# Princic-1837592/julia-raytracer

Measured on AMD Instinct MI355X. Metric: Mrays/s + wall-clock render time, cornellbox 1280×720×256spp, higher is better.
Workload: dtype f32; 1 GPU; cornellbox path 1280x720x256spp; scene=cornellbox, sampler=path, width=1280, height=720, spp=256, bounces=8, batch=256, traversal=near, traversal_requested=auto, bvh=middle, parallelism=1 tile groups x 1 sample ranges + RCCL reduce

## Files before the change

julia-raytracer_amd/csrc/jt_kernels.h:

```cpp
#pragma once

#include <hip/hip_runtime.h>

#include <algorithm>

#include "jt_bsdf.h"
#include "jt_device.h"
#include "jt_push.h"

#ifndef JT_STAMPS
#define JT_STAMPS 0
#endif
#ifndef JT_NODE_REPEAT_NONE
#define JT_NODE_REPEAT_NONE 4
#endif
#ifndef JT_NODE_REPEAT
#define JT_NODE_REPEAT 3
#endif
#ifndef JT_FIRST_POP_NONE
#define JT_FIRST_POP_NONE 1
#endif
#ifndef JT_FIRST_POP
#define JT_FIRST_POP 2
#endif
// ... 1026 lines not shown
    p[9 * BLOCK] = p[9 * BLOCK] * omw + tn.z * aw;
}

template <int F, class AovT>
__device__ __forceinline__ bool path_hit(const DScene& S, const DParams& P, Path& st, Hit isec, const AovT& aov,
                                         unsigned& shades) {
    if (!isec.hit) {
        if (st.bounce() > 0 || !P.envhidden)
            st.set_radiance<F>(st.radiance<F>() + st.weight<F>() * eval_environment<F>(S, st.d));
        return true;
    }
    bool in_volume = false;
    if ((F & FT_VOL) && st.flag(F_VOLUME)) {
        float rl = rand1f(st.rng), rd = rand1f(st.rng);
        float distance = sample_transmittance(st.vol.density, isec.t, rl, rd);
        v3 tr = eval_transmittance(st.vol.density, distance);
        float tp = sample_transmittance_pdf(st.vol.density, distance, isec.t);
        st.set_weight<F>((st.weight<F>() * tr) / tp);
        in_volume = distance < isec.t;
        isec.t = distance;
    }
    if (!in_volume) {
        v3 outgoing = -st.d;
        Shading sh;
        eval_shading<F>(S, isec.inst, isec.elem, V2(isec.u, isec.v), outgoing, sh);
        shades++;
        if (P.nocaustics) {
            st.set_max_roughness<F>(jl_max(sh.mat.roughness, st.max_roughness<F>()));
            sh.mat.roughness = st.max_roughness<F>();
        }
        if ((F & FT_OPAC) && sh.mat.opacity < 1 && rand1f(st.rng) >= sh.mat.opacity) {
            if (st.opbounce() > 128) return true;
            st.ctl += 1u << CTL_OPB;
            st.o = sh.position + st.d * 0.01f;
            return next_bounce_retry(P, st);
        }
        if (st.bounce() == 0) {
            st.set_flag(F_HIT);
            aov_update<F>(aov, sh.mat.color, sh.normal);
        }
        st.set_radiance<F>(st.radiance<F>() + st.weight<F>() * (dot(sh.normal, outgoing) >= 0 ? sh.mat.emission : V3(0, 0, 0)));
        v3 incoming;
        const bool delta = is_delta(sh.mat);
        if (!delta) {
            if (rand1f(st.rng) < 0.5f) {
                float rnl = rand1f(st.rng);
                v2 rn = rand2f(st.rng);
                incoming = sample_bsdfcos<F>(sh.mat, sh.normal, outgoing, rnl, rn);
            } else {
                float rl = rand1f(st.rng), rel = rand1f(st.rng);
                v2 ruv = rand2f(st.rng);
                incoming = sample_lights<F>(S, sh.position, rl, rel, ruv);
            }
            if (is_zero(incoming)) return true;
#if JT_FUSED_BSDF
            v3 fb;
            float pbv;
            eval_bsdfcos_pdf<F>(sh.mat, sh.normal, outgoing, incoming, fb, pbv);
            st.set_weight<F>(st.weight<F>() * fb);
            st.set_pb<F>(pbv);
#else
            st.set_weight<F>(st.weight<F>() * eval_bsdfcos<F>(sh.mat, sh.normal, outgoing, incoming));
            st.set_pb<F>(sample_bsdfcos_pdf<F>(sh.mat, sh.normal, outgoing, incoming));
#endif
        } else {
            float rnl = rand1f(st.rng);
            incoming = sample_delta<F>(sh.mat, sh.normal, outgoing, rnl);
            v3 f = eval_delta<F>(sh.mat, sh.normal, outgoing, incoming);
            float pd = sample_delta_pdf<F>(sh.mat, sh.normal, outgoing, incoming);
            st.set_weight<F>((st.weight<F>() * f) / pd);
        }
        const int mtype = sh.mat.type;
        if ((F & FT_VOL) && (mtype == M_REFRACTIVE || mtype == M_VOLUMETRIC || mtype == M_SUBSURFACE) &&
            dot(sh.normal, outgoing) * dot(sh.normal, incoming) < 0) {
            if (!st.flag(F_VOLUME)) {
                st.set_flag(F_VOLUME);
                st.vol.density = sh.mat.density;
                st.vol.scattering = sh.mat.scattering;
                st.vol.scanisotropy = sh.mat.scanisotropy;
            } else {
                st.clear_flag(F_VOLUME);
            }
        }
        st.o = sh.position;
        st.d = incoming;
        return delta ? after_weight<F>(P, st) : begin_light_pdf<F>(S, P, st);
    }
    v3 outgoing = -st.d;
    v3 position = st.o + st.d * isec.t;
    v3 incoming;
    if (rand1f(st.rng) < 0.5f) {
        (void)rand1f(st.rng);
        v2 rn = rand2f(st.rng);
        incoming = sample_scattering(st.vol, outgoing, rn);
    } else {
        float rl = rand1f(st.rng), rel = rand1f(st.rng);
        v2 ruv = rand2f(st.rng);
        incoming = sample_lights<F>(S, position, rl, rel, ruv);
    }
    if (is_zero(incoming)) return true;
    st.set_weight<F>(st.weight<F>() * eval_scattering(st.vol, outgoing, incoming));
    st.set_pb<F>(sample_scattering_pdf(st.vol, outgoing, incoming));
    st.o = position;
    st.d = incoming;
    return begin_light_pdf<F>(S, P, st);
}

template <int F, class AovT>
__device__ __forceinline__ bool naive_hit(const DScene& S, const DParams& P, Path& st, Hit isec, const AovT& aov,
                                          unsigned& shades) {
    if (!isec.hit) {
        if (st.bounce() > 0 || !P.envhidden)
            st.set_radiance<F>(st.radiance<F>() + st.weight<F>() * eval_environment<F>(S, st.d));
        return true;
    }
    v3 outgoing = -st.d;
    Shading sh;
    eval_shading<F>(S, isec.inst, isec.elem, V2(isec.u, isec.v), outgoing, sh);
    shades++;
    if ((F & FT_OPAC) && sh.mat.opacity < 1 && rand1f(st.rng) >= sh.mat.opacity) {
        if (st.opbounce() > 128) return true;
        st.ctl += 1u << CTL_OPB;
        st.o = sh.position + st.d * 0.01f;
        return next_bounce_retry(P, st);
    }
    if (st.bounce() == 0) {
        st.set_flag(F_HIT);
        aov_update<F>(aov, sh.mat.color, sh.normal);
    }
    st.set_radiance<F>(st.radiance<F>() + st.weight<F>() * (dot(sh.normal, outgoing) >= 0 ? sh.mat.emission : V3(0, 0, 0)));
    v3 incoming, f;
    float p;
    if (sh.mat.roughness != 0) {
        float rnl = rand1f(st.rng);
        v2 rn = rand2f(st.rng);
        incoming = sample_bsdfcos<F>(sh.mat, sh.normal, outgoing, rnl, rn);
        if (is_zero(incoming)) return true;
#if JT_FUSED_BSDF
        eval_bsdfcos_pdf<F>(sh.mat, sh.normal, outgoing, incoming, f, p);
#else
        f = eval_bsdfcos<F>(sh.mat, sh.normal, outgoing, incoming);
        p = sample_bsdfcos_pdf<F>(sh.mat, sh.normal, outgoing, incoming);
#endif
    } else {
        float rnl = rand1f(st.rng);
        incoming = sample_delta<F>(sh.mat, sh.normal, outgoing, rnl);
        if (is_zero(incoming)) return true;
        f = eval_delta<F>(sh.mat, sh.normal, outgoing, incoming);
        p = sample_delta_pdf<F>(sh.mat, sh.normal, outgoing, incoming);
    }
    st.set_weight<F>((st.weight<F>() * f) / p);
    st.o = sh.position;
    st.d = incoming;
    return after_weight<F>(P, st);
}

__device__ __forceinline__ void eval_camera(const DCamera& cam, v2 image_uv, v2 lens_uv, v3& ro, v3& rd) {
    const fr3 frame = frame_from(cam.frame);
    const v2 film = V2(cam.film_x, cam.film_y);
    if (!cam.orthographic) {
        v3 q = V3(film.x * (0.5f - image_uv.x), film.y * (image_uv.y - 0.5f), cam.lens);
        v3 dc = -normalize(q);
        v3 e = V3(lens_uv.x * cam.aperture / 2, lens_uv.y * cam.aperture / 2, 0);
        v3 p = (dc * cam.focus) / __builtin_fabsf(dc.z);
        v3 d = normalize(p - e);
        ro = transform_point(frame, e);
        rd = transform_direction(frame, d);
    } else {
        float scale = 1 / cam.lens;
        v3 q = V3(film.x * (0.5f - image_uv.x) * scale, film.y * (image_uv.y - 0.5f) * scale, cam.lens);
        v3 e = V3(-q.x, -q.y, 0) + V3(lens_uv.x * cam.aperture / 2, lens_uv.y * cam.aperture / 2, 0);
        v3 p = V3(-q.x, -q.y, -cam.focus);
        v3 d = normalize(p - e);
        ro = transform_point(frame, e);
        rd = transform_direction(frame, d);
    }
}

template <int F>
__device__ __forceinline__ void start_path(const DParams& P, int i, int j, int pixel, int sample, Path& st) {
    st.rng = rng_init(P.seed, pixel, sample);
    v2 puv = rand2f(st.rng);
    v2 luv = rand2f(st.rng);
    v2 uv;
    if (!P.tentfilter) {
        uv = V2(((float)i + puv.x) / (float)P.width, ((float)j + puv.y) / (float)P.height);
    } else {
        const float width = 2.0f, offset = 0.5f;
        v2 fuv = V2(width * (puv.x < 0.5f ? __builtin_sqrtf(2 * puv.x) - 1 : 1 - __builtin_sqrtf(2 - 2 * puv.x)) + offset,
                    width * (puv.y < 0.5f ? __builtin_sqrtf(2 * puv.y) - 1 : 1 - __builtin_sqrtf(2 - 2 * puv.y)) + offset);
        uv = V2(((float)i + fuv.x) / (float)P.width, ((float)j + fuv.y) / (float)P.height);
    }
    eval_camera(P.cam, uv, P.cam.pinhole ? sample_disk_signs(luv) : sample_disk(luv), st.o, st.d);
    st.set_radiance<F>(V3(0, 0, 0));
    st.set_weight<F>(V3(1, 1, 1));
    st.set_max_roughness<F>(0.0f);
    st.ctl = 0u;
    st.phase = PH_SCENE;
}

__device__ __forceinline__ int lane_count(unsigned long long m) {
    return __builtin_popcount((unsigned)m) + __builtin_popcount((unsigned)(m >> 32));
}

__device__ __forceinline__ unsigned wave_sum(unsigned v) {
    for (int off = 32; off > 0; off >>= 1) v += __shfl_xor(v, off, 64);
    return v;
}

struct DAccum {
    float4* image;
    float4* albedo;
    float4* normal;
    long long* hits;
    unsigned long long* counters;
    unsigned* work;
    float4* part_img;
    float4* part_alb;
    float4* part_nrm;
    int nslot;
};

struct KArgs {
    DScene S;
    DParams P;
    int s_begin, s_end;
    DAccum A;
};
#ifndef JT_KARG_RELOAD
#define JT_KARG_RELOAD 1
#endif
template <int F>
__host__ __device__ constexpr bool karg_reload() {
    return JT_KARG_RELOAD && (F & ~(FT_LINL | FT_NOIL)) != (FT_TEX | FT_ATTR | FT_MAT | FT_OPAC | FT_XFORM | FT_ENV | FT_QUAD);
}
template <class T>
__device__ __forceinline__ T karg(size_t off) {
    typedef __attribute__((address_space(4))) const char* kptr;
    kptr p = (kptr)__builtin_amdgcn_kernarg_segment_ptr();
    asm volatile("" : "+s"(p));
    return *(const __attribute__((address_space(4))) T*)(p + off);
}
#ifndef JT_KARG_SCENE
#define JT_KARG_SCENE 1
#endif
template <bool NCACHE, int F>
__host__ __device__ constexpr bool karg_scene() {
    return NCACHE && JT_KARG_SCENE && (F & ~(FT_LINL | FT_NOIL)) != (FT_TEX | FT_ATTR | FT_MAT | FT_OPAC | FT_XFORM);
}
template <bool FROM_KARG>
__device__ __forceinline__ const DScene& shade_scene(const DScene& S) {
    if constexpr (FROM_KARG) {
        typedef __attribute__((address_space(4))) const char* kptr;
        kptr p = (kptr)__builtin_amdgcn_kernarg_segment_ptr();
        asm volatile("" : "+s"(p));
        return *(const DScene*)(const __attribute__((address_space(4))) DScene*)(p + offsetof(KArgs, S));
    } else {
        return S;
    }
}
#ifndef JT_KARG_PARAMS
#define JT_KARG_PARAMS 1
#endif
template <int SAMPLER, int F>
__host__ __device__ constexpr bool karg_params_on() {
    return JT_KARG_PARAMS && SAMPLER == 1 && (F & ~(FT_LINL | FT_NOIL)) != (FT_TEX | FT_ATTR | FT_MAT | FT_OPAC | FT_XFORM);
}
template <bool FROM_KARG>
__device__ __forceinline__ const DParams& karg_params(const DParams& P) {
    if constexpr (FROM_KARG) {
        typedef __attribute__((address_space(4))) const char* kptr;
        kptr p = (kptr)__builtin_amdgcn_kernarg_segment_ptr();
        asm volatile("" : "+s"(p));
        return *(const DParams*)(const __attribute__((address_space(4))) DParams*)(p + offsetof(KArgs, P));
    } else {
        return P;
    }
}
#ifndef JT_KARG_SCENE_LDS
#define JT_KARG_SCENE_LDS 1
#endif
__device__ __forceinline__ DScene blob_scene(const DScene& S, const uint4* blob);
__host__ __device__ constexpr size_t lds_stack_bytes(bool ovf, int ring, int need);
template <bool NCACHE, int RING, bool OVF, int F>
__device__ __forceinline__ DScene shade_scene_lds(const DScene& S0) {
    if constexpr (!NCACHE && JT_KARG_SCENE_LDS) {
        extern __shared__ uint4 dyn_lds[];
        const DScene& K = shade_scene<true>(S0);
        return blob_scene(K, dyn_lds + lds_stack_bytes(OVF, RING, K.stack_need) / 16);
    } else {
        return S0;
    }
}
#define JT_A(f) (karg_reload<F>() ? karg<decltype(DAccum::f)>(offsetof(KArgs, A) + offsetof(DAccum, f)) : A.f)
#define JT_SB (karg_reload<F>() ? karg<int>(offsetof(KArgs, s_begin)) : s_begin)
#define JT_SE (karg_reload<F>() ? karg<int>(offsetof(KArgs, s_end)) : s_end)

constexpr int NBANDS = 8, BAND_STRIDE = 16;

__host__ __device__ __forceinline__ int launch_tiles(const DParams& P) {
    return plan_tiles(P.width, P.height, P.tile_stride, P.tile_offset);
}

#ifndef JT_ITEM_FIRST_POP
#define JT_ITEM_FIRST_POP 2
#endif
template <bool WIDE, int F>
__host__ __device__ constexpr bool item_first_pop() {
    return JT_ITEM_FIRST_POP == 1 || (JT_ITEM_FIRST_POP == 2 && !WIDE && !ft_none(F));
}
constexpr unsigned ITEM_NONE = 0xffffffffu;

__device__ __forceinline__ int item_pixel(unsigned item, const DParams& P, int tiles_x) {
    const int t = (int)(item >> 6), l = (int)(item & 63u);
    return ((t / tiles_x) * 8 + (l >> 3)) * P.width + (t % tiles_x) * 8 + (l & 7);
}
__host__ __device__ __forceinline__ int item_slot(unsigned item, const DParams& P) {
    const int t = (int)(item >> 6);
    float inv = 1.0f / (float)P.tile_stride;
#if defined(__HIP_DEVICE_COMPILE__)
    inv = __uint_as_float(__builtin_amdgcn_readfirstlane(__float_as_uint(inv)));
#endif
    const int u = (int)((float)(t - P.tile_offset) * inv + 0.5f);
    return u * 64 + (int)(item & 63u);
}
__device__ __forceinline__ float stream_weight(const DParams& P, int s) {
    return 1.0f / (float)(((s - P.first) >> P.lk) + 1);
}

#if JT_STAMPS
#define JT_STAMP(x) x
#else
#define JT_STAMP(x)
#endif

template <int SAMPLER, int RING, bool OVF, int COUNT, int F, bool NCACHE, bool WIDE>
__device__ __forceinline__ void trace_body_items(const DScene& S0, const DParams& P0, int s_begin, int s_end,
                                                 const DAccum& A, int* stack) {
    const DScene& S = S0;
    const DParams& P = P0;
    static_assert(lane_lds(F), "the per-lane item body keeps the lane's sample index in LDS");
    const int lane = threadIdx.x & 63;
    const int oslot = (int)blockIdx.x * BLOCK + (int)threadIdx.x;
    if constexpr ((F & (FT_TEX | FT_ENV)) != 0) {
        for (int k = threadIdx.x; k < 512; k += BLOCK) tex_lut[k] = k < 256 ? S.srgb_lut[k] : S.byte_lut[k - 256];
        __syncthreads();
    }
    Counters cnt{0, 0, 0, 0};
    constexpr bool WC = !ft_none(F);
    unsigned w_paths = 0, w_rays = 0, w_lq = 0;
    __shared__ unsigned wave_cnt[WC ? 1 : (BLOCK / 64) * 4];
    unsigned* const wcnt = wave_cnt + (WC ? 0 : (threadIdx.x >> 6) * 4);
    if (!WC && lane < 3) wcnt[lane] = 0u;
    auto lds_count = [&](int k, bool c) {
        if (c) __hip_atomic_fetch_add(wcnt + k, 1u, __ATOMIC_RELAXED, __HIP_MEMORY_SCOPE_WORKGROUP);
    };
    __shared__ float acc_lds[acc_slots(F) * BLOCK];
    float* acc = acc_lds + threadIdx.x;
    int* const acc_i = reinterpret_cast<int*>(acc);
#if JT_STAMPS
    unsigned long long t_trav = 0, t_shade = 0, n_trav = 0, n_shade = 0, lanes_p = 0, lanes_n = 0, steps_p = 0, steps_n = 0;
    unsigned long long t_hit = 0, t_fin = 0, t_qb = 0, n_phit = 0, n_fin = 0, idle = 0, n_mph = 0, n_mty = 0, n_mid = 0;
    unsigned long long lanes_sh = 0, lanes_hit = 0, t_start = 0, n_start = 0, lanes_start = 0;
#endif
    const int tiles_x = (P.width + 7) / 8, tiles = launch_tiles(P);
    const int kstr = 1 << P.lk;
    const int nq = s_end - s_begin < kstr ? s_end - s_begin : kstr;
    unsigned xcc;
    asm volatile("s_getreg_b32 %0, hwreg(HW_REG_XCC_ID)" : "=s"(xcc));
    int band_k = 0;
    int ut = 0, uq = 0, bnext = 64;
    bool drained = false;
    unsigned item = ITEM_NONE;
    bool next_sample = false;
    Aov aov{acc, 0.0f, P.first, P.lk};
    Path st;
    st.pk = acc + acc_base_slots(F) * BLOCK;
    Trav T;
    T.sp = -1;
    T.nprim = 0;
    T.nxt = W_EMPTY;
    for (;;) {
        JT_STAMP(const unsigned long long ts0 = __builtin_amdgcn_s_memtime());
        bool start = next_sample;
        for (;;) {
            const unsigned long long needm = __builtin_amdgcn_ballot_w64(item == ITEM_NONE);
            if (!needm || drained) break;
            if (bnext >= 64) {
                const int band = (int)((xcc + (unsigned)band_k) & (NBANDS - 1));
                constexpr int STRIP = JT_BAND_STRIP;
                const int gx = tiles_x % P.tile_stride == 0 ? tiles_x / P.tile_stride : 0;
                const bool strips = STRIP > 1 && gx > 0;
                const int tiles_y = (P.height + 7) / 8;
                const int bt0 = strips ? band * tiles_y / NBANDS * gx : band * tiles / NBANDS;
                const int bn = strips ? (band + 1) * tiles_y / NBANDS * gx - bt0 : (band + 1) * tiles / NBANDS - bt0;
                unsigned unit = 0;
                if (lane == 0) unit = atomicAdd(JT_A(work) + band * BAND_STRIDE, 1u);
                unit = __builtin_amdgcn_readfirstlane(unit);
                if (unit >= (unsigned)bn * (unsigned)nq) {
                    if (++band_k >= NBANDS) drained = true;
                    continue;
                }
                uq = (int)(unit % (unsigned)nq);
                const int tu = (int)(unit / (unsigned)nq);
                int tile = bt0 + tu;
                if (strips) {
                    const int rows = bn / gx, sidx = tu / (STRIP * gx);
                    const int v = tu - sidx * STRIP * gx, h = rows - sidx * STRIP < STRIP ? rows - sidx * STRIP : STRIP;
                    tile = bt0 + (sidx * STRIP + v % h) * gx + v / h;
                }
                ut = tile * P.tile_stride + P.tile_offset;
                bnext = 0;
            }
            const int nneed = lane_count(needm), take = nneed < 64 - bnext ? nneed : 64 - bnext;
            const int rank = (int)__builtin_amdgcn_mbcnt_hi((unsigned)(needm >> 32), __builtin_amdgcn_mbcnt_lo((unsigned)needm, 0u));
            if (item == ITEM_NONE && rank < take) {
                const int l = bnext + rank;
                const int i = (ut % tiles_x) * 8 + (l & 7), j = (ut / tiles_x) * 8 + (l >> 3);
                if (i < P.width && j < P.height) {
                    item = (unsigned)(ut * 64 + l);
                    start = true;
                    const int s = JT_SB + uq;
                    acc_i[11 * BLOCK] = s;
                    const int pixel = j * P.width + i;
                    float4 im = make_float4(0, 0, 0, 0), al = im, nr = im;
                    int h = 0;
                    if (s - P.first >= kstr) {
                        if (P.lk == 0) {
                            im = JT_A(image)[pixel];
                            al = JT_A(albedo)[pixel];
                            nr = JT_A(normal)[pixel];
                            h = (int)JT_A(hits)[pixel];
                        } else {
                            const size_t o = (size_t)((s - P.first) & (kstr - 1)) * (size_t)JT_A(nslot) +
                                             (size_t)item_slot(item, P);
                            im = JT_A(part_img)[o];
                            al = JT_A(part_alb)[o];
                            nr = JT_A(part_nrm)[o];
                            h = __float_as_int(al.w);
                        }
                    }
                    acc[0] = im.x;
                    acc[BLOCK] = im.y;
                    acc[2 * BLOCK] = im.z;
                    acc[3 * BLOCK] = im.w;
                    acc[4 * BLOCK] = al.x;
                    acc[5 * BLOCK] = al.y;
                    acc[6 * BLOCK] = al.z;
                    acc[7 * BLOCK] = nr.x;
                    acc[8 * BLOCK] = nr.y;
                    acc[9 * BLOCK] = nr.z;
                    acc_i[10 * BLOCK] = h;
                }
            }
            bnext += take;
        }
        next_sample = false;
        if (start) {
            const int sample = acc_i[11 * BLOCK];
            const int pixel = item_pixel(item, P, tiles_x);
            if (!ft_none(F)) acc[12 * BLOCK] = stream_weight(P, sample);
            const DParams& P = karg_params<karg_params_on<SAMPLER, F>()>(P0);
            start_path<F>(P, pixel % P.width, pixel / P.width, pixel, sample, st);
            query_start<WIDE>(S, T, st.o, st.d, -1, stack);
            if (!WC) lds_count(1, true);
            if constexpr (item_first_pop<WIDE, F>()) {
#pragma unroll
                for (int k = 0; k < (!ft_none(F) && (F & FT_LINL) ? JT_FIRST_POP : JT_FIRST_POP_NONE); k++)
                    if (wants_node<WIDE>(T)) node_step_any<WIDE, RING, OVF, COUNT, NCACHE, F>(S, T, stack, oslot, cnt);
            }
        }
        if (WC) w_rays += lane_count(__builtin_amdgcn_ballot_w64(start));
#if JT_STAMPS
        const unsigned long long ts1 = __builtin_amdgcn_s_memtime();
        t_start += ts1 - ts0;
        n_start++;
        lanes_start += lane_count(__builtin_amdgcn_ballot_w64(start));
#endif
        if (__builtin_amdgcn_ballot_w64(item != ITEM_NONE) == 0) break;
        constexpr bool LSTEP = light_steps(SAMPLER, F);
        for (;;) {
            const bool wantp = T.nprim > 0;
            const bool wantn = wants_node<WIDE>(T);
            const bool waiting = query_done<WIDE>(T);
            const int np = lane_count(__builtin_amdgcn_ballot_w64(wantp));
            const int nn = lane_count(__builtin_amdgcn_ballot_w64(wantn));
            int nw = lane_count(__builtin_amdgcn_ballot_w64(waiting));
            const int nb = np + nn;
            if (LSTEP && !S.light_inline) {
                const bool wantl = waiting && st.phase == PH_LIGHT;
                const int nl = lane_count(__builtin_amdgcn_ballot_w64(wantl));
                if (nl > 0 && (nl >= P.light_lanes || nb == 0)) {
                    bool c_lq = false, c_ray = false;
                    if (wantl && rerun_tie<WIDE>(S, T, st.o, st.d, S.lights[st.li].instance, stack)) {
                    } else if (wantl) {
                        if (light_hit<F>(S, P, st, query_hit(T))) {
                            st.phase = PH_FINISH;
                        } else if (st.phase == PH_LIGHT) {
                            if (WC) c_lq = true;
                            else lds_count(2, true);
                            query_start<WIDE>(S, T, st.o, st.d, S.lights[st.li].instance, stack);
                        } else {
                            if (WC) c_ray = true;
                            else lds_count(1, true);
                            query_start<WIDE>(S, T, st.o, st.d, -1, stack);
                        }
                    }
                    if (WC) {
                        w_lq += lane_count(__builtin_amdgcn_ballot_w64(c_lq));
                        w_rays += lane_count(__builtin_amdgcn_ballot_w64(c_ray));
                    }
                    continue;
                }
                nw -= nl;
            }
            if (nb == 0 || nw >= (nb + nw < P.wait_lanes ? nb + nw : P.wait_lanes)) break;
#if JT_STAMPS
            n_trav++;
            idle += 64 - lane_count(__builtin_amdgcn_ballot_w64(item != ITEM_NONE));
            if (np * JT_VOTE_P >= nn * JT_VOTE_N) { steps_p++; lanes_p += np; } else { steps_n++; lanes_n += nn; }
#endif
            if (JT_RAY_FROM_PATH && !(F & FT_XFORM)) {
                T.lo = st.o;
                T.ld = st.d;
            }
            if (np * JT_VOTE_P >= nn * JT_VOTE_N) {
                if (T.nprim > 0) prim_step<COUNT, F>(S, T, cnt);
            } else {
                constexpr int NREP = ft_none(F) ? JT_NODE_REPEAT_NONE : JT_NODE_REPEAT;
#pragma unroll
                for (int k = 0; k < NREP; k++)
                    if (wants_node<WIDE>(T)) node_step_any<WIDE, RING, OVF, COUNT, NCACHE, F>(S, T, stack, oslot, cnt);
            }
        }
#if JT_STAMPS
        const unsigned long long ts2 = __builtin_amdgcn_s_memtime();
        t_trav += ts2 - ts1;
        n_shade++;
        lanes_sh += lane_count(__builtin_amdgcn_ballot_w64(query_done<WIDE>(T)));
        {
            int mid = -1, mt = -1;
            if (query_done<WIDE>(T) && st.phase == PH_SCENE && T.h_inst >= 0) {
                mid = S.inst_shade[T.h_inst].material;
                mt = (F & FT_MAT) ? S.materials[mid].type : (int)M_MATTE;
            }
            if (__builtin_amdgcn_ballot_w64(mt >= 0)) {
                n_mph++;
                lanes_hit += lane_count(__builtin_amdgcn_ballot_w64(mt >= 0));
                for (int ty = 0; ty <= (int)M_GLTFPBR; ty++) n_mty += __builtin_amdgcn_ballot_w64(mt == ty) ? 1u : 0u;
                bool counted = mt < 0;
                for (;;) {
                    const unsigned long long m = __builtin_amdgcn_ballot_w64(!counted);
                    if (!m) break;
                    const int v = __shfl(mid, __ffsll((long long)m) - 1);
                    counted = counted || mid == v;
                    n_mid++;
                }
            }
        }
        unsigned long long ts3 = ts2, ts4 = ts2;
#endif
        constexpr bool LINL = (F & (FT_LINL | FT_NOIL)) != 0;
        {
            const bool tie = query_done<WIDE>(T) && (T.nh & (TIE_SEEN | REF_RERUN)) == TIE_SEEN &&
                             !(LSTEP && st.phase == PH_FINISH);
            if (S.order_flip && __builtin_amdgcn_ballot_w64(tie))
                if (tie) rerun_tie<WIDE>(S, T, st.o, st.d, SAMPLER == 1 && !LINL && st.phase == PH_LIGHT ? S.lights[st.li].instance : -1, stack);
        }
        bool c_path = false, c_lq = false, c_ray = false;
        unsigned n_inl = 0;
        if (query_done<WIDE>(T)) {
            const DParams& P = karg_params<karg_params_on<SAMPLER, F>()>(P0);
            const DScene SL = shade_scene_lds<NCACHE, RING, OVF, F>(S0);
            const DScene& S = NCACHE ? shade_scene<karg_scene<NCACHE, F>()>(S0) : SL;
            bool alive = true;
            const bool light = SAMPLER == 1 && !LINL && st.phase == PH_LIGHT;
            bool done;
            if (LSTEP && st.phase == PH_FINISH) done = true;
            else if (light) done = light_hit<F>(S, P, st, query_hit(T));
            else if (SAMPLER == 2) done = naive_hit<F>(S, P, st, query_hit(T), aov, cnt.shades);
            else done = path_hit<F>(S, P, st, query_hit(T), aov, cnt.shades);
            bool chained = false;
            if (SAMPLER == 1 && !done && st.phase == PH_LIGHT && chains_inline(F, S)) {
                unsigned nlq = 0;
                chained = true;
                done = light_chain<WIDE, RING, OVF, COUNT, NCACHE, F>(S, P, st, T, stack, oslot, cnt, [&] {
                    if (WC) nlq++;
                    else lds_count(2, true);
                });
                if (WC) n_inl += nlq;
            }
#if JT_STAMPS
            ts3 = __builtin_amdgcn_s_memtime();
            n_phit++;
#endif
            if (done) {
                if (WC) c_path = true;
                else lds_count(0, true);
                v3 radiance = st.radiance<F>();
                if (!all_finite(radiance)) radiance = V3(0, 0, 0);
                const float mr = max3(radiance);
                if (mr > P.clamp) radiance = radiance * (P.clamp / mr);
                const float w = aov.w<F>();
                const float omw = 1 - w;
                const bool hit = st.flag(F_HIT);
                const bool env = !hit && !P.envhidden && S.nenvs != 0;
                const v4 target = (hit || env) ? V4(radiance.x, radiance.y, radiance.z, 1) : V4(0, 0, 0, 0);
                if (!hit) aov_update<F>(aov, env ? V3(1, 1, 1) : V3(0, 0, 0), -st.d);
                acc[0] = acc[0] * omw + target.x * w;
                acc[BLOCK] = acc[BLOCK] * omw + target.y * w;
                acc[2 * BLOCK] = acc[2 * BLOCK] * omw + target.z * w;
                acc[3 * BLOCK] = acc[3 * BLOCK] * omw + target.w * w;
                if (hit || env) acc_i[10 * BLOCK] += 1;
                alive = false;
                T.sp = -1;
                const int sample = acc_i[11 * BLOCK];
                if (sample + kstr >= JT_SE) {
                    const int pixel = item_pixel(item, P, tiles_x);
                    const float4 im = make_float4(acc[0], acc[BLOCK], acc[2 * BLOCK], acc[3 * BLOCK]);
                    if (P.lk == 0) {
                        JT_A(image)[pixel] = im;
                        JT_A(albedo)[pixel] = make_float4(acc[4 * BLOCK], acc[5 * BLOCK], acc[6 * BLOCK], 0.0f);
                        JT_A(normal)[pixel] = make_float4(acc[7 * BLOCK], acc[8 * BLOCK], acc[9 * BLOCK], 0.0f);
                        JT_A(hits)[pixel] = (long long)acc_i[10 * BLOCK];
                    } else {
                        const size_t o = (size_t)((sample - P.first) & (kstr - 1)) * (size_t)JT_A(nslot) +
                                         (size_t)item_slot(item, P);
                        JT_A(part_img)[o] = im;
                        JT_A(part_alb)[o] = make_float4(acc[4 * BLOCK], acc[5 * BLOCK], acc[6 * BLOCK], __int_as_float(acc_i[10 * BLOCK]));
                        JT_A(part_nrm)[o] = make_float4(acc[7 * BLOCK], acc[8 * BLOCK], acc[9 * BLOCK], 0.0f);
                    }
                    item = ITEM_NONE;
                } else {
                    acc_i[11 * BLOCK] = sample + kstr;
                    next_sample = true;
                }
            }
#if JT_STAMPS
            ts4 = __builtin_amdgcn_s_memtime();
            if (__builtin_amdgcn_ballot_w64(done)) n_fin++;
#endif
            if (alive) {
                if (SAMPLER == 1 && !LINL && st.phase == PH_LIGHT) {
                    if (WC) c_lq = true;
                    else lds_count(2, true);
                    query_start<WIDE>(S, T, st.o, st.d, S.lights[st.li].instance, stack);
                } else {
                    if (WC) c_ray = true;
                    else lds_count(1, true);
                    if (SAMPLER == 1 && chain_dinv_once<WIDE, OVF, NCACHE, F>() && __builtin_amdgcn_ballot_w64(!chained) == 0)
                        query_restart<F>(S, T, st.o, st.d, stack);
                    else query_start<WIDE>(S, T, st.o, st.d, -1, stack);
                }
#pragma unroll
                for (int k = 0; k < (!ft_none(F) && (F & FT_LINL) ? JT_FIRST_POP : JT_FIRST_POP_NONE); k++)
                    if (wants_node<WIDE>(T)) node_step_any<WIDE, RING, OVF, COUNT, NCACHE, F>(S, T, stack, oslot, cnt);
            }
        }
#if JT_STAMPS
        const unsigned long long ts5 = __builtin_amdgcn_s_memtime();
        t_shade += ts5 - ts2;
        t_hit += ts3 - ts2;
        t_fin += ts4 - ts3;
        t_qb += ts5 - ts4;
#endif
        if (WC) {
            w_paths += lane_count(__builtin_amdgcn_ballot_w64(c_path));
            w_lq += lane_count(__builtin_amdgcn_ballot_w64(c_lq));
            w_rays += lane_count(__builtin_amdgcn_ballot_w64(c_ray));
            if (SAMPLER == 1 && chains_inline(F, S)) w_lq += __builtin_amdgcn_readfirstlane(wave_sum(n_inl));
        }
    }
#if JT_STAMPS
    if (lane == 0) {
        unsigned long long* dbg = A.counters + 8;
        const unsigned long long v[24] = {t_trav, t_shade, n_trav,  n_shade, lanes_p, lanes_n,  steps_p, steps_n,
                                          0,      t_hit,   t_fin,   t_qb,    0,       n_phit,   n_fin,   idle,
                                          n_mph,  n_mty,   n_mid,   lanes_sh, lanes_hit, t_start, n_start, lanes_start};
        for (int k = 0; k < 24; k++) atomicAdd(dbg + k, v[k]);
    }
#endif
    const unsigned wv[3] = {w_paths, w_rays, w_lq};
    unsigned v[7] = {0u, 0u, 0u, cnt.nodes, cnt.instances, cnt.prims, COUNT ? cnt.shades : 0u};
#pragma unroll
    for (int k = 0; k < 7; k++) {
        unsigned sum = k < 3 ? (WC ? wv[k] : wcnt[k]) : wave_sum(v[k]);
        if (lane == 0 && sum) atomicAdd(&A.counters[k], (unsigned long long)sum);
    }
}

struct DCombine {
    float w[JT_MAX_STREAMS];
    int ns;
};
inline void combine_weights(long long n, int lk, DCombine& cw) {
    cw = DCombine{};
    cw.ns = combine_weights(n, lk, cw.w);
}
#ifndef JT_WAVES
#define JT_WAVES 0
#endif
#ifndef JT_WAVES_NONE
#define JT_WAVES_NONE 5
#endif
#if JT_WAVES > 0
#define JT_WAVES_PER_EU __attribute__((amdgpu_waves_per_eu(JT_WAVES, JT_WAVES)))
#define JT_WAVES_PER_EU_F(F) \
    __attribute__((amdgpu_waves_per_eu(ft_none(F) ? JT_WAVES_NONE : JT_WAVES, ft_none(F) ? JT_WAVES_NONE : JT_WAVES)))
#else
#define JT_WAVES_PER_EU
#define JT_WAVES_PER_EU_F(F)
#endif
__host__ __device__ constexpr size_t lds_stack_bytes(bool ovf, int ring, int need) {
    return (size_t)(ovf ? ring : need) * BLOCK * 4;
}

__device__ __forceinline__ DScene blob_scene(const DScene& S, const uint4* blob) {
    DScene L = S;
    L.nodes = reinterpret_cast<const DNode*>(blob + S.o_nodes);
    L.wnodes = reinterpret_cast<const DWide*>(blob + S.o_wnodes);
    L.prims = reinterpret_cast<const float4*>(blob + S.o_prims);
    L.inst_trav = reinterpret_cast<const DInstTrav*>(blob + S.o_inst_trav);
    L.inst_blas = reinterpret_cast<const int4*>(blob + S.o_inst_blas);
    L.inst_shade = reinterpret_cast<const DInstShade*>(blob + S.o_inst_shade);
    L.shapes = reinterpret_cast<const DShape*>(blob + S.o_shapes);
    L.pos = reinterpret_cast<const float4*>(blob + S.o_pos);
    L.nrm = reinterpret_cast<const float4*>(blob + S.o_nrm);
    L.tc = reinterpret_cast<const float2*>(blob + S.o_tc);
    L.col = reinterpret_cast<const float4*>(blob + S.o_col);
    L.elems = reinterpret_cast<const int4*>(blob + S.o_elems);
    L.enrm = reinterpret_cast<const float4*>(blob + S.o_enrm);
    L.enrm_id = reinterpret_cast<const float4*>(blob + S.o_enrm_id);
    L.materials = reinterpret_cast<const DMaterial*>(blob + S.o_materials);
    L.lights = reinterpret_cast<const DLight*>(blob + S.o_lights);
    L.light_hit = reinterpret_cast<const int4*>(blob + S.o_light_hit);
    L.light_elems = reinterpret_cast<const float4*>(blob + S.o_light_elems);
    L.cdf = reinterpret_cast<const float*>(blob + S.o_cdf);
    return L;
}

template <int SAMPLER, int RING, bool OVF, int COUNT, int F, bool WIDE>
__global__ __launch_bounds__(BLOCK) JT_WAVES_PER_EU void trace_kernel(DScene S, DParams P, int s_begin, int s_end, DAccum A) {
    __shared__ int lds_stack[RING * BLOCK];
    trace_body_items<SAMPLER, RING, OVF, COUNT, F, true, WIDE>(S, P, s_begin, s_end, A, lds_stack + threadIdx.x);
}

template <int SAMPLER, int RING, bool OVF, int COUNT, int F, bool WIDE>
__global__ __launch_bounds__(BLOCK) JT_WAVES_PER_EU_F(F) void trace_kernel_lds(DScene S, DParams P, int s_begin, int s_end, DAccum A) {
    extern __shared__ uint4 dyn_lds[];
    uint4* blob = dyn_lds + lds_stack_bytes(OVF, RING, S.stack_need) / 16;
    for (int k = threadIdx.x; k < S.blob_n16; k += BLOCK) blob[k] = S.blob[k];
    __syncthreads();
    const DScene L = blob_scene(S, blob);
    trace_body_items<SAMPLER, RING, OVF, COUNT, F, false, WIDE>(L, P, s_begin, s_end, A, reinterpret_cast<int*>(dyn_lds) + threadIdx.x);
}

template <int SAMPLER, int RING, bool OVF, int COUNT, int F, bool LDSK, bool WIDE>
hipError_t launch_t(const DScene& S, const DParams& P, int s0, int s1, const DAccum& A, hipStream_t st, int cus) {
    const long long units = (long long)launch_tiles(P) * std::min(s1 - s0, 1 << P.lk);
    const int want = (int)std::min<long long>((units + BLOCK / 64 - 1) / (BLOCK / 64), 1 << 30);
    if (want == 0) return hipSuccess;
    int per_cu = 0;
    hipError_t e;
    if constexpr (LDSK) {
        if (S.blob_n16 > 0) {
        const size_t lds = lds_stack_bytes(OVF, RING, S.stack_need) + (size_t)S.blob_n16 * 16;
        const void* k = (const void*)trace_kernel_lds<SAMPLER, RING, OVF, COUNT, F, WIDE>;
        if ((e = hipFuncSetAttribute(k, hipFuncAttributeMaxDynamicSharedMemorySize, (int)lds)) != hipSuccess) return e;
        if (hipOccupancyMaxActiveBlocksPerMultiprocessor(&per_cu, k, BLOCK, lds) != hipSuccess || per_cu < 1) per_cu = 1;
        const int nwg = std::min(want, std::min(per_cu, 8) * cus);
        hipLaunchKernelGGL((trace_kernel_lds<SAMPLER, RING, OVF, COUNT, F, WIDE>), dim3(nwg), dim3(BLOCK), lds, st, S, P, s0, s1, A);
        return hipGetLastError();
        }
    }
    const void* k = (const void*)trace_kernel<SAMPLER, RING, OVF, COUNT, F, WIDE>;
    if (hipOccupancyMaxActiveBlocksPerMultiprocessor(&per_cu, k, BLOCK, 0) != hipSuccess || per_cu < 1) per_cu = 1;
    const int nwg = std::min(want, std::min(per_cu, 8) * cus);
    hipLaunchKernelGGL((trace_kernel<SAMPLER, RING, OVF, COUNT, F, WIDE>), dim3(nwg), dim3(BLOCK), 0, st, S, P, s0, s1, A);
    return hipGetLastError();
}

constexpr int FT_MESH = FT_TEX | FT_ATTR | FT_MAT | FT_OPAC | FT_XFORM;
constexpr int FT_MESH_ENV = FT_MESH | FT_ENV;
constexpr int FT_MESH_ENV_QUAD = FT_MESH_ENV | FT_QUAD;
inline int kernel_mask(int feat, int need, int ring, bool lds, bool linl, bool inst_light) {
    if (need <= 16) return feat == FT_NONE ? (linl ? FT_NONE | FT_LINL : FT_NONE) : FT_ALL;
    if (ring > 16 || lds) return FT_ALL;
    for (int m : {FT_MESH | FT_LINL, FT_MESH_ENV | FT_NOIL, FT_MESH_ENV_QUAD | FT_LINL})
        if (!(feat & ~m & ~(FT_LINL | FT_NOIL)) && ((m & FT_LINL) ? linl : !inst_light)) return m;
    return FT_ALL;
}

constexpr int NUM_BASE_CONFIGS = 8;
template <int ID>
struct LaunchConfig;
#define JT_LAUNCH_CONFIG(ID, R, O, F, L)                            \
    template <>                                                      \
    struct LaunchConfig<ID> {                                        \
        static constexpr int ring = R;                               \
        static constexpr bool ovf = O;                               \
        static constexpr int feat = F;                               \
        static constexpr bool lds = L;                               \
        static constexpr bool wide = false;                          \
    };                                                               \
    template <>                                                      \
    struct LaunchConfig<ID + NUM_BASE_CONFIGS> : LaunchConfig<ID> {  \
        static constexpr bool wide = true;                           \
    };
JT_LAUNCH_CONFIG(0, 16, false, FT_NONE | FT_LINL, true)
JT_LAUNCH_CONFIG(1, 16, false, FT_ALL, true)
JT_LAUNCH_CONFIG(2, 16, true, FT_MESH | FT_LINL, false)
JT_LAUNCH_CONFIG(3, 16, true, FT_MESH_ENV | FT_NOIL, false)
JT_LAUNCH_CONFIG(4, 16, true, FT_MESH_ENV_QUAD | FT_LINL, false)
JT_LAUNCH_CONFIG(5, 16, true, FT_ALL, true)
JT_LAUNCH_CONFIG(6, 32, true, FT_ALL, true)
JT_LAUNCH_CONFIG(7, 16, false, FT_NONE, true)
#undef JT_LAUNCH_CONFIG
constexpr int NUM_LAUNCH_CONFIGS = 2 * NUM_BASE_CONFIGS;

template <int ID, int SAMPLER, int COUNT>
hipError_t launch_cfg(const DScene& S, const DParams& P, int s0, int s1, const DAccum& A, hipStream_t st, int cus) {
    using C = LaunchConfig<ID>;
    return launch_t<SAMPLER, C::ring, C::ovf, COUNT, C::feat, C::lds, C::wide>(S, P, s0, s1, A, st, cus);
}
#define JT_KV_FOR(ID, KW)                                                                                    \
    KW hipError_t launch_cfg<ID, 1, 0>(const DScene&, const DParams&, int, int, const DAccum&, hipStream_t, int); \
    KW hipError_t launch_cfg<ID, 1, 1>(const DScene&, const DParams&, int, int, const DAccum&, hipStream_t, int); \
    KW hipError_t launch_cfg<ID, 2, 0>(const DScene&, const DParams&, int, int, const DAccum&, hipStream_t, int); \
    KW hipError_t launch_cfg<ID, 2, 1>(const DScene&, const DParams&, int, int, const DAccum&, hipStream_t, int);

}
```

julia-raytracer_amd/csrc/jt_plan.h:

```cpp
#pragma once

#if defined(__HIPCC__) || defined(__CUDACC__)
#define JT_PLAN_HD __host__ __device__ inline
#else
#define JT_PLAN_HD inline
#endif

#define JT_STREAMS_MIN 16
#define JT_STREAMS_WIDE 32
#define JT_STREAM_ITEMS (1LL << 22)
#define JT_STREAM_ITEMS_MAX (1LL << 27)
#ifndef JT_MAX_STREAMS
#define JT_MAX_STREAMS 64
#endif

namespace jtk {

JT_PLAN_HD int plan_tiles(int width, int height, int stride, int offset) {
    const int all = ((width + 7) / 8) * ((height + 7) / 8);
    return all > offset ? (all - offset + stride - 1) / stride : 0;
}

struct SlotPixel {
    int i, j;
    bool inside;
};
JT_PLAN_HD SlotPixel slot_pixel(int g, int width, int height, int tile_stride, int tile_offset) {
    const int tiles_x = (width + 7) / 8;
    const int t = (g >> 6) * tile_stride + tile_offset, l = g & 63;
    const int i = (t % tiles_x) * 8 + (l & 7), j = (t / tiles_x) * 8 + (l >> 3);
    return SlotPixel{i, j, i < width && j < height};
}

JT_PLAN_HD long long traced_pixels(int width, int height, int stride, int offset) {
    const int tiles = plan_tiles(width, height, stride, offset);
    long long n = 0;
    for (int u = 0; u < tiles; u++) {
        const SlotPixel p = slot_pixel(u * 64, width, height, stride, offset);
        const int w = width - p.i, h = height - p.j;
        n += (long long)(w < 8 ? w : 8) * (h < 8 ? h : 8);
    }
    return n;
}

JT_PLAN_HD int stream_log2(long long pixels, int batch) {
    if (batch <= 1) return 0;
    long long want = batch >= 2 * JT_STREAMS_WIDE ? JT_STREAMS_WIDE : JT_STREAMS_MIN;
    while (pixels * want < JT_STREAM_ITEMS) want *= 2;
    int lk = 0;
    while (lk < 6 && (2LL << lk) <= want && (2 << lk) <= batch && (2 << lk) <= JT_MAX_STREAMS &&
           pixels * (2LL << lk) <= JT_STREAM_ITEMS_MAX)
        lk++;
    return lk;
}

JT_PLAN_HD int combine_weights(long long n, int lk, float* w) {
    const long long k = 1LL << lk;
    const int ns = (int)(n < k ? n : k);
    for (int j = 0; j < ns; j++) w[j] = (float)((double)((n - 1 - j) / k + 1) / (double)n);
    return ns;
}

JT_PLAN_HD int chunk_samples(long long nslot) {
    int m = JT_MAX_STREAMS;
    while (m > 1 && 2 * nslot * m > JT_STREAM_ITEMS_MAX) m >>= 1;
    return m;
}

JT_PLAN_HD void sample_share(int s0, int s1, int d, int D, int* a, int* b) {
    const long long L = s1 - s0;
    *a = s0 + (int)(L * d / D);
    *b = s0 + (int)(L * (d + 1) / D);
}

}
```

Before: 12500 Mrays/s.

## Refill work items after shading and issue rays from one merged query site

Moves the work-fetch and path-start block from the top of the persistent loop to after shading. New paths and continuing bounces then share a single query_start/first-pop site (ISSUE=1) instead of two separate divergent call sites. Item encoding switches to a bit-packed tile-row/column form so pixel coordinates come from shifts and masks rather than integer division by tiles_x. The aim is less divergence and fewer duplicated traversal-start instances per iteration, at the cost of a reordered loop and a new item encoding that item_slot must decode consistently.

```diff
diff --git a/julia-raytracer_amd/csrc/jt_kernels.h b/julia-raytracer_amd/csrc/jt_kernels.h
--- a/julia-raytracer_amd/csrc/jt_kernels.h
+++ b/julia-raytracer_amd/csrc/jt_kernels.h
@@ -1352,21 +1352,17 @@
     return plan_tiles(P.width, P.height, P.tile_stride, P.tile_offset);
 }
 
-#ifndef JT_ITEM_FIRST_POP
-#define JT_ITEM_FIRST_POP 2
-#endif
-template <bool WIDE, int F>
-__host__ __device__ constexpr bool item_first_pop() {
-    return JT_ITEM_FIRST_POP == 1 || (JT_ITEM_FIRST_POP == 2 && !WIDE && !ft_none(F));
+#ifndef JT_ISSUE_ONCE
+#define JT_ISSUE_ONCE 1
+#endif
+template <int SAMPLER, bool WIDE, int F>
+__host__ __device__ constexpr int issue_once() {
+    return JT_ISSUE_ONCE;
 }
 constexpr unsigned ITEM_NONE = 0xffffffffu;
 
-__device__ __forceinline__ int item_pixel(unsigned item, const DParams& P, int tiles_x) {
-    const int t = (int)(item >> 6), l = (int)(item & 63u);
-    return ((t / tiles_x) * 8 + (l >> 3)) * P.width + (t % tiles_x) * 8 + (l & 7);
-}
 __host__ __device__ __forceinline__ int item_slot(unsigned item, const DParams& P) {
-    const int t = (int)(item >> 6);
+    const int t = item_tile(item, P.width);
     float inv = 1.0f / (float)P.tile_stride;
 #if defined(__HIP_DEVICE_COMPILE__)
     inv = __uint_as_float(__builtin_amdgcn_readfirstlane(__float_as_uint(inv)));
@@ -1411,7 +1407,7 @@
 #if JT_STAMPS
     unsigned long long t_trav = 0, t_shade = 0, n_trav = 0, n_shade = 0, lanes_p = 0, lanes_n = 0, steps_p = 0, steps_n = 0;
     unsigned long long t_hit = 0, t_fin = 0, t_qb = 0, n_phit = 0, n_fin = 0, idle = 0, n_mph = 0, n_mty = 0, n_mid = 0;
-    unsigned long long lanes_sh = 0, lanes_hit = 0, t_start = 0, n_start = 0, lanes_start = 0;
+    unsigned long long lanes_sh = 0, lanes_hit = 0, t_start = 0, n_start = 0, lanes_start = 0, t_hand = 0;
 #endif
     const int tiles_x = (P.width + 7) / 8, tiles = launch_tiles(P);
     const int kstr = 1 << P.lk;
@@ -1419,10 +1415,11 @@
     unsigned xcc;
     asm volatile("s_getreg_b32 %0, hwreg(HW_REG_XCC_ID)" : "=s"(xcc));
     int band_k = 0;
-    int ut = 0, uq = 0, bnext = 64;
+    unsigned ubase = 0;
+    int uq = 0, bnext = 64;
     bool drained = false;
     unsigned item = ITEM_NONE;
-    bool next_sample = false;
+    constexpr int ISSUE = issue_once<SAMPLER, WIDE, F>();
     Aov aov{acc, 0.0f, P.first, P.lk};
     Path st;
     st.pk = acc + acc_base_slots(F) * BLOCK;
@@ -1432,102 +1429,6 @@
     T.nxt = W_EMPTY;
     for (;;) {
         JT_STAMP(const unsigned long long ts0 = __builtin_amdgcn_s_memtime());
-        bool start = next_sample;
-        for (;;) {
-            const unsigned long long needm = __builtin_amdgcn_ballot_w64(item == ITEM_NONE);
-            if (!needm || drained) break;
-            if (bnext >= 64) {
-                const int band = (int)((xcc + (unsigned)band_k) & (NBANDS - 1));
-                constexpr int STRIP = JT_BAND_STRIP;
-                const int gx = tiles_x % P.tile_stride == 0 ? tiles_x / P.tile_stride : 0;
-                const bool strips = STRIP > 1 && gx > 0;
-                const int tiles_y = (P.height + 7) / 8;
-                const int bt0 = strips ? band * tiles_y / NBANDS * gx : band * tiles / NBANDS;
-                const int bn = strips ? (band + 1) * tiles_y / NBANDS * gx - bt0 : (band + 1) * tiles / NBANDS - bt0;
-                unsigned unit = 0;
-                if (lane == 0) unit = atomicAdd(JT_A(work) + band * BAND_STRIDE, 1u);
-                unit = __builtin_amdgcn_readfirstlane(unit);
-                if (unit >= (unsigned)bn * (unsigned)nq) {
-                    if (++band_k >= NBANDS) drained = true;
-                    continue;
-                }
-                uq = (int)(unit % (unsigned)nq);
-                const int tu = (int)(unit / (unsigned)nq);
-                int tile = bt0 + tu;
-                if (strips) {
-                    const int rows = bn / gx, sidx = tu / (STRIP * gx);
-                    const int v = tu - sidx * STRIP * gx, h = rows - sidx * STRIP < STRIP ? rows - sidx * STRIP : STRIP;
-                    tile = bt0 + (sidx * STRIP + v % h) * gx + v / h;
-                }
-                ut = tile * P.tile_stride + P.tile_offset;
-                bnext = 0;
-            }
-            const int nneed = lane_count(needm), take = nneed < 64 - bnext ? nneed : 64 - bnext;
-            const int rank = (int)__builtin_amdgcn_mbcnt_hi((unsigned)(needm >> 32), __builtin_amdgcn_mbcnt_lo((unsigned)needm, 0u));
-            if (item == ITEM_NONE && rank < take) {
-                const int l = bnext + rank;
-                const int i = (ut % tiles_x) * 8 + (l & 7), j = (ut / tiles_x) * 8 + (l >> 3);
-                if (i < P.width && j < P.height) {
-                    item = (unsigned)(ut * 64 + l);
-                    start = true;
-                    const int s = JT_SB + uq;
-                    acc_i[11 * BLOCK] = s;
-                    const int pixel = j * P.width + i;
-                    float4 im = make_float4(0, 0, 0, 0), al = im, nr = im;
-                    int h = 0;
-                    if (s - P.first >= kstr) {
-                        if (P.lk == 0) {
-                            im = JT_A(image)[pixel];
-                            al = JT_A(albedo)[pixel];
-                            nr = JT_A(normal)[pixel];
-                            h = (int)JT_A(hits)[pixel];
-                        } else {
-                            const size_t o = (size_t)((s - P.first) & (kstr - 1)) * (size_t)JT_A(nslot) +
-                                             (size_t)item_slot(item, P);
-                            im = JT_A(part_img)[o];
-                            al = JT_A(part_alb)[o];
-                            nr = JT_A(part_nrm)[o];
-                            h = __float_as_int(al.w);
-                        }
-                    }
-                    acc[0] = im.x;
-                    acc[BLOCK] = im.y;
-                    acc[2 * BLOCK] = im.z;
-                    acc[3 * BLOCK] = im.w;
-                    acc[4 * BLOCK] = al.x;
-                    acc[5 * BLOCK] = al.y;
-                    acc[6 * BLOCK] = al.z;
-                    acc[7 * BLOCK] = nr.x;
-                    acc[8 * BLOCK] = nr.y;
-                    acc[9 * BLOCK] = nr.z;
-                    acc_i[10 * BLOCK] = h;
-                }
-            }
-            bnext += take;
-        }
-        next_sample = false;
-        if (start) {
-            const int sample = acc_i[11 * BLOCK];
-            const int pixel = item_pixel(item, P, tiles_x);
-            if (!ft_none(F)) acc[12 * BLOCK] = stream_weight(P, sample);
-            const DParams& P = karg_params<karg_params_on<SAMPLER, F>()>(P0);
-            start_path<F>(P, pixel % P.width, pixel / P.width, pixel, sample, st);
-            query_start<WIDE>(S, T, st.o, st.d, -1, stack);
-            if (!WC) lds_count(1, true);
-            if constexpr (item_first_pop<WIDE, F>()) {
-#pragma unroll
-                for (int k = 0; k < (!ft_none(F) && (F & FT_LINL) ? JT_FIRST_POP : JT_FIRST_POP_NONE); k++)
-                    if (wants_node<WIDE>(T)) node_step_any<WIDE, RING, OVF, COUNT, NCACHE, F>(S, T, stack, oslot, cnt);
-            }
-        }
-        if (WC) w_rays += lane_count(__builtin_amdgcn_ballot_w64(start));
-#if JT_STAMPS
-        const unsigned long long ts1 = __builtin_amdgcn_s_memtime();
-        t_start += ts1 - ts0;
-        n_start++;
-        lanes_start += lane_count(__builtin_amdgcn_ballot_w64(start));
-#endif
-        if (__builtin_amdgcn_ballot_w64(item != ITEM_NONE) == 0) break;
         constexpr bool LSTEP = light_steps(SAMPLER, F);
         for (;;) {
             const bool wantp = T.nprim > 0;
@@ -1585,7 +1486,7 @@
         }
 #if JT_STAMPS
         const unsigned long long ts2 = __builtin_amdgcn_s_memtime();
-        t_trav += ts2 - ts1;
+        t_trav += ts2 - ts0;
         n_shade++;
         lanes_sh += lane_count(__builtin_amdgcn_ballot_w64(query_done<WIDE>(T)));
         {
@@ -1619,18 +1520,19 @@
         }
         bool c_path = false, c_lq = false, c_ray = false;
         unsigned n_inl = 0;
+        bool go = false;
+        bool start = false;
+        bool chained = false;
         if (query_done<WIDE>(T)) {
             const DParams& P = karg_params<karg_params_on<SAMPLER, F>()>(P0);
             const DScene SL = shade_scene_lds<NCACHE, RING, OVF, F>(S0);
             const DScene& S = NCACHE ? shade_scene<karg_scene<NCACHE, F>()>(S0) : SL;
-            bool alive = true;
             const bool light = SAMPLER == 1 && !LINL && st.phase == PH_LIGHT;
             bool done;
             if (LSTEP && st.phase == PH_FINISH) done = true;
             else if (light) done = light_hit<F>(S, P, st, query_hit(T));
             else if (SAMPLER == 2) done = naive_hit<F>(S, P, st, query_hit(T), aov, cnt.shades);
             else done = path_hit<F>(S, P, st, query_hit(T), aov, cnt.shades);
-            bool chained = false;
             if (SAMPLER == 1 && !done && st.phase == PH_LIGHT && chains_inline(F, S)) {
                 unsigned nlq = 0;
                 chained = true;
@@ -1662,11 +1564,11 @@
                 acc[2 * BLOCK] = acc[2 * BLOCK] * omw + target.z * w;
                 acc[3 * BLOCK] = acc[3 * BLOCK] * omw + target.w * w;
                 if (hit || env) acc_i[10 * BLOCK] += 1;
-                alive = false;
                 T.sp = -1;
                 const int sample = acc_i[11 * BLOCK];
                 if (sample + kstr >= JT_SE) {
-                    const int pixel = item_pixel(item, P, tiles_x);
+                    const SlotPixel px = item_pixel(item, P.width, P.height);
+                    const int pixel = px.j * P.width + px.i;
                     const float4 im = make_float4(acc[0], acc[BLOCK], acc[2 * BLOCK], acc[3 * BLOCK]);
                     if (P.lk == 0) {
                         JT_A(image)[pixel] = im;
@@ -1683,49 +1585,160 @@
                     item = ITEM_NONE;
                 } else {
                     acc_i[11 * BLOCK] = sample + kstr;
-                    next_sample = true;
+                    start = true;
                 }
+            } else {
+                go = true;
             }
 #if JT_STAMPS
             ts4 = __builtin_amdgcn_s_memtime();
             if (__builtin_amdgcn_ballot_w64(done)) n_fin++;
 #endif
-            if (alive) {
-                if (SAMPLER == 1 && !LINL && st.phase == PH_LIGHT) {
-                    if (WC) c_lq = true;
-                    else lds_count(2, true);
-                    query_start<WIDE>(S, T, st.o, st.d, S.lights[st.li].instance, stack);
-                } else {
-                    if (WC) c_ray = true;
-                    else lds_count(1, true);
-                    if (SAMPLER == 1 && chain_dinv_once<WIDE, OVF, NCACHE, F>() && __builtin_amdgcn_ballot_w64(!chained) == 0)
-                        query_restart<F>(S, T, st.o, st.d, stack);
-                    else query_start<WIDE>(S, T, st.o, st.d, -1, stack);
-                }
-#pragma unroll
-                for (int k = 0; k < (!ft_none(F) && (F & FT_LINL) ? JT_FIRST_POP : JT_FIRST_POP_NONE); k++)
-                    if (wants_node<WIDE>(T)) node_step_any<WIDE, RING, OVF, COUNT, NCACHE, F>(S, T, stack, oslot, cnt);
-            }
+        }
+        if (WC) {
+            w_paths += lane_count(__builtin_amdgcn_ballot_w64(c_path));
+            if (SAMPLER == 1 && chains_inline(F, S)) w_lq += __builtin_amdgcn_readfirstlane(wave_sum(n_inl));
         }
 #if JT_STAMPS
         const unsigned long long ts5 = __builtin_amdgcn_s_memtime();
         t_shade += ts5 - ts2;
         t_hit += ts3 - ts2;
         t_fin += ts4 - ts3;
-        t_qb += ts5 - ts4;
+#endif
+        for (;;) {
+            const unsigned long long needm = __builtin_amdgcn_ballot_w64(item == ITEM_NONE);
+            if (!needm || drained) break;
+            if (bnext >= 64) {
+                const int band = (int)((xcc + (unsigned)band_k) & (NBANDS - 1));
+                constexpr int STRIP = JT_BAND_STRIP;
+                const int gx = tiles_x % P.tile_stride == 0 ? tiles_x / P.tile_stride : 0;
+                const bool strips = STRIP > 1 && gx > 0;
+                const int tiles_y = (P.height + 7) / 8;
+                const int bt0 = strips ? band * tiles_y / NBANDS * gx : band * tiles / NBANDS;
+                const int bn = strips ? (band + 1) * tiles_y / NBANDS * gx - bt0 : (band + 1) * tiles / NBANDS - bt0;
+                unsigned unit = 0;
+                if (lane == 0) unit = atomicAdd(JT_A(work) + band * BAND_STRIDE, 1u);
+                unit = __builtin_amdgcn_readfirstlane(unit);
+                if (unit >= (unsigned)bn * (unsigned)nq) {
+                    if (++band_k >= NBANDS) drained = true;
+                    continue;
+                }
+                uq = (int)(unit % (unsigned)nq);
+                const int tu = (int)(unit / (unsigned)nq);
+                int tile = bt0 + tu;
+                if (strips) {
+                    const int rows = bn / gx, sidx = tu / (STRIP * gx);
+                    const int v = tu - sidx * STRIP * gx, h = rows - sidx * STRIP < STRIP ? rows - sidx * STRIP : STRIP;
+                    tile = bt0 + (sidx * STRIP + v % h) * gx + v / h;
+                }
+                ubase = item_base(tile * P.tile_stride + P.tile_offset, P.width);
+                bnext = 0;
+            }
+            const int nneed = lane_count(needm), take = nneed < 64 - bnext ? nneed : 64 - bnext;
+            const int rank = (int)__builtin_amdgcn_mbcnt_hi((unsigned)(needm >> 32), __builtin_amdgcn_mbcnt_lo((unsigned)needm, 0u));
+            if (item == ITEM_NONE && rank < take) {
+                const unsigned it = ubase + (unsigned)(bnext + rank);
+                const SlotPixel px = item_pixel(it, P.width, P.height);
+                if (px.inside) {
+                    item = it;
+                    start = true;
+                    const int s = JT_SB + uq;
+                    acc_i[11 * BLOCK] = s;
+                    const int pixel = px.j * P.width + px.i;
+                    float4 im = make_float4(0, 0, 0, 0), al = im, nr = im;
+                    int h = 0;
+                    if (s - P.first >= kstr) {
+                        if (P.lk == 0) {
+                            im = JT_A(image)[pixel];
+                            al = JT_A(albedo)[pixel];
+                            nr = JT_A(normal)[pixel];
+                            h = (int)JT_A(hits)[pixel];
+                        } else {
+                            const size_t o = (size_t)((s - P.first) & (kstr - 1)) * (size_t)JT_A(nslot) +
+                                             (size_t)item_slot(item, P);
+                            im = JT_A(part_img)[o];
+                            al = JT_A(part_alb)[o];
+                            nr = JT_A(part_nrm)[o];
+                            h = __float_as_int(al.w);
+                        }
+                    }
+                    acc[0] = im.x;
+                    acc[BLOCK] = im.y;
+                    acc[2 * BLOCK] = im.z;
+                    acc[3 * BLOCK] = im.w;
+                    acc[4 * BLOCK] = al.x;
+                    acc[5 * BLOCK] = al.y;
+                    acc[6 * BLOCK] = al.z;
+                    acc[7 * BLOCK] = nr.x;
+                    acc[8 * BLOCK] = nr.y;
+                    acc[9 * BLOCK] = nr.z;
+                    acc_i[10 * BLOCK] = h;
+                }
+            }
+            bnext += take;
+        }
+#if JT_STAMPS
+        const unsigned long long ts6 = __builtin_amdgcn_s_memtime();
+        t_hand += ts6 - ts5;
+        n_start++;
+        lanes_start += lane_count(__builtin_amdgcn_ballot_w64(start));
+#endif
+        if (__builtin_amdgcn_ballot_w64(item != ITEM_NONE) == 0) break;
+        if (start) {
+            const int sample = acc_i[11 * BLOCK];
+            if (!ft_none(F)) acc[12 * BLOCK] = stream_weight(P, sample);
+            const DParams& P = karg_params<karg_params_on<SAMPLER, F>()>(P0);
+            const SlotPixel px = item_pixel(item, P.width, P.height);
+            start_path<F>(P, px.i, px.j, px.j * P.width + px.i, sample, st);
+            if constexpr (ISSUE == 0) {
+                query_start<WIDE>(S, T, st.o, st.d, -1, stack);
+                if (!WC) lds_count(1, true);
+                if constexpr (!WIDE && !ft_none(F)) {
+#pragma unroll
+                    for (int k = 0; k < (!ft_none(F) && (F & FT_LINL) ? JT_FIRST_POP : JT_FIRST_POP_NONE); k++)
+                        if (wants_node<WIDE>(T)) node_step_any<WIDE, RING, OVF, COUNT, NCACHE, F>(S, T, stack, oslot, cnt);
+                }
+            } else if constexpr (ISSUE == 2 && SAMPLER == 1 && chain_dinv_once<WIDE, OVF, NCACHE, F>()) {
+                T.wdinv = V3(jl_rcp(st.d.x), jl_rcp(st.d.y), jl_rcp(st.d.z));
+                if (!(F & FT_XFORM)) T.negmask = neg_mask(st.d, S.order_flip);
+                chained = true;
+            } else {
+                chained = false;
+            }
+        }
+        if (WC && ISSUE == 0) w_rays += lane_count(__builtin_amdgcn_ballot_w64(start));
+        JT_STAMP(const unsigned long long ts7 = __builtin_amdgcn_s_memtime());
+        if (ISSUE != 0 ? (go || start) : go) {
+            if (SAMPLER == 1 && !LINL && st.phase == PH_LIGHT) {
+                if (WC) c_lq = true;
+                else lds_count(2, true);
+                query_start<WIDE>(S, T, st.o, st.d, S.lights[st.li].instance, stack);
+            } else {
+                if (WC) c_ray = true;
+                else lds_count(1, true);
+                if (SAMPLER == 1 && chain_dinv_once<WIDE, OVF, NCACHE, F>() && __builtin_amdgcn_ballot_w64(!chained) == 0)
+                    query_restart<F>(S, T, st.o, st.d, stack);
+                else query_start<WIDE>(S, T, st.o, st.d, -1, stack);
+            }
+#pragma unroll
+            for (int k = 0; k < (!ft_none(F) && (F & FT_LINL) ? JT_FIRST_POP : JT_FIRST_POP_NONE); k++)
+                if (wants_node<WIDE>(T)) node_step_any<WIDE, RING, OVF, COUNT, NCACHE, F>(S, T, stack, oslot, cnt);
+        }
+#if JT_STAMPS
+        const unsigned long long ts8 = __builtin_amdgcn_s_memtime();
+        t_start += ts7 - ts6;
+        t_qb += ts8 - ts7;
 #endif
         if (WC) {
-            w_paths += lane_count(__builtin_amdgcn_ballot_w64(c_path));
             w_lq += lane_count(__builtin_amdgcn_ballot_w64(c_lq));
             w_rays += lane_count(__builtin_amdgcn_ballot_w64(c_ray));
-            if (SAMPLER == 1 && chains_inline(F, S)) w_lq += __builtin_amdgcn_readfirstlane(wave_sum(n_inl));
         }
     }
 #if JT_STAMPS
     if (lane == 0) {
         unsigned long long* dbg = A.counters + 8;
         const unsigned long long v[24] = {t_trav, t_shade, n_trav,  n_shade, lanes_p, lanes_n,  steps_p, steps_n,
-                                          0,      t_hit,   t_fin,   t_qb,    0,       n_phit,   n_fin,   idle,
+                                          t_hand, t_hit,   t_fin,   t_qb,    0,       n_phit,   n_fin,   idle,
                                           n_mph,  n_mty,   n_mid,   lanes_sh, lanes_hit, t_start, n_start, lanes_start};
         for (int k = 0; k < 24; k++) atomicAdd(dbg + k, v[k]);
     }
diff --git a/julia-raytracer_amd/csrc/jt_plan.h b/julia-raytracer_amd/csrc/jt_plan.h
--- a/julia-raytracer_amd/csrc/jt_plan.h
+++ b/julia-raytracer_amd/csrc/jt_plan.h
@@ -29,6 +29,24 @@
     const int tiles_x = (width + 7) / 8;
     const int t = (g >> 6) * tile_stride + tile_offset, l = g & 63;
     const int i = (t % tiles_x) * 8 + (l & 7), j = (t / tiles_x) * 8 + (l >> 3);
+    return SlotPixel{i, j, i < width && j < height};
+}
+
+JT_PLAN_HD int item_shift(int width) {
+    const unsigned tiles_x = (unsigned)(width + 7) / 8u;
+    return tiles_x > 1u ? 6 + 32 - __builtin_clz(tiles_x - 1u) : 6;
+}
+JT_PLAN_HD unsigned item_base(int t, int width) {
+    const int tiles_x = (width + 7) / 8;
+    return ((unsigned)(t / tiles_x) << item_shift(width)) | ((unsigned)(t % tiles_x) << 6);
+}
+JT_PLAN_HD int item_tile(unsigned item, int width) {
+    const int shift = item_shift(width), tiles_x = (width + 7) / 8;
+    return (int)(item >> shift) * tiles_x + (int)((item >> 6) & ((1u << (shift - 6)) - 1u));
+}
+JT_PLAN_HD SlotPixel item_pixel(unsigned item, int width, int height) {
+    const int shift = item_shift(width), l = (int)(item & 63u);
+    const int i = (int)((item >> 6) & ((1u << (shift - 6)) - 1u)) * 8 + (l & 7), j = (int)(item >> shift) * 8 + (l >> 3);
     return SlotPixel{i, j, i < width && j < height};
 }
 
```

After: 12590 Mrays/s (median of 6 runs). No clear change (+0.7%).
